# Monash-Connected-Autonomous-Vehicle/unsupervised-pseuso-LiDAR

Measured on AMD Instinct MI355X. Metric: images/sec (fwd+bwd) KITTI 192x640 triplets, full training step, higher is better.
Workload: dtype f32; 1 GPU; BASELINE.json configs[1]: per-GPU batch=12, 192x640 KITTI-shaped triplets, ResNet-18 depth encoder + 6-DoF PoseNet, fp32 (the ResNet trunk's 3x3 stride-1 convolutions and their data gradients: fp32 contractions on split operands -- three bf16 planes per operand, six bf16-MFMA plane products, fp32 accumulation; every other launch: fp32 MFMA), one step = 2x depth fwd + pose fwd + warp/L1/smooth loss; global_batch=12, parallelism=dp1

## Files before the change

### include/mcav_conv.h

```cpp
#ifndef MCAV_CONV_H
#define MCAV_CONV_H

#include <stddef.h>
#include <stdint.h>

#ifdef __cplusplus
extern "C" {
#endif

#define MCAV_G_DIRECT 0
#define MCAV_G_SMALLC 1
#define MCAV_G_ADJ_REFLECT 2
#define MCAV_G_ADJ_STRIDE2 3

#define MCAV_PAD_ZERO 0
#define MCAV_PAD_REFLECT 1

#define MCAV_ACT_NONE 0
#define MCAV_ACT_RELU 1
#define MCAV_ACT_ELU 2
#define MCAV_ACT_SIGMOID 3

#define MCAV_DACT_AFTER_ADDEND 0x100

// ... 35 lines not shown
    int B, Hs, Ws, C1, C2, up1;
    int kh, kw, Kp;
    int mode, stride, sign, offset, pad_mode;
    const float* dy;
    int Hd, Wd, Cdy, dy_choff;
    int Cout, Cin;
    float* dw_oihw;
    int accumulate;
    float* dbias;
    int tile;
    int upm, Cin_total, ci_offset;
    int mma;
} mcav_wgrad_desc;

size_t mcav_wgrad_workspace_bytes(const mcav_wgrad_desc* d);
int mcav_wgrad_uses_bf16(const mcav_wgrad_desc* d);
int mcav_wgrad(const mcav_wgrad_desc* d, void* workspace, size_t workspace_bytes, void* stream);

typedef struct mcav_wgrad_reduce_item {
    const float* slab;
    float* pre;
    float* dw;
    float* dbias;
    unsigned long long elems;
    int splits, groups, per_group, Ktot, slabN, Kp, taps, Cout, Cin, ci_t, accumulate, upm, cin_total, ci_off;
    int pre_bx, red_gx, red_gy, pre_first, red_first, reserved;
} mcav_wgrad_reduce_item;
int mcav_wgrad_deferred(const mcav_wgrad_desc* d, void* workspace, size_t workspace_bytes, mcav_wgrad_reduce_item* item, void* stream);
int mcav_wgrad_reduce_plan(mcav_wgrad_reduce_item* items, int n, int* presum_blocks, int* reduce_blocks, size_t* lds_bytes);
int mcav_wgrad_reduce_multi(const mcav_wgrad_reduce_item* items_dev, int n, int presum_blocks, int reduce_blocks, size_t lds_bytes, void* stream);

int mcav_pack_weights(const float* w_oihw, int Cout, int Cin, int kh, int kw, int transposed, float* packed, int Np, int Kp,
                      void* stream);

int mcav_pack_weights_multi(const void* items_dev, int nitems, int nblocks, void* stream);
int mcav_f32_to_bf16(const float* src, void* dst_bf16, size_t n, void* stream);
int mcav_f32_to_bf16_planes(const float* src, void* dst_bf16, size_t n, void* stream);
int mcav_pack_weights_blocks(int taps, int transposed, int Np, int Kp);
int mcav_pack_stem_weights(const float* w_oihw, int Cout, int Cin, float* packed, void* stream);
int mcav_pack_weights_upmerge(const float* w_oihw, int Cout, int Cin, int C1, float* packed, int Np, void* stream);
int mcav_pack_weights_upmerge_adj(const float* w_oihw, int Cout, int Cin, int C1, float* packed, int Np, int Kp, void* stream);
// ... 82 lines not shown
```

### unsupervised-pseuso-lidar_amd/csrc/conv_igemm.hip

```cpp
#include <stdlib.h>
#include <map>
#include <mutex>
#include <type_traits>
#include <utility>

#include "conv_shared.h"
#include "kernel_timer.h"

namespace mcav {

template <class T, int KIND>
__global__ __launch_bounds__(256) void igemm_kernel(IgemmParams p) {
    constexpr int BM = T::BM, BN = T::BN;
    constexpr int CK = T::KD;
    __shared__ __attribute__((aligned(16))) float As[2][BM][T::LD];
    __shared__ __attribute__((aligned(16))) float Bs[2][BN][T::LD];
    __shared__ int s_out[BM];
    __shared__ float s_stat[T::WAVES_M][2][BN];
    constexpr int MAXTAB = 9;
    __shared__ unsigned s_o1[KIND == K_GENERIC ? 1 : MAXTAB][KIND == K_GENERIC ? 1 : BM];
    __shared__ unsigned s_o2[KIND == K_GENERIC ? 1 : MAXTAB][KIND == K_GENERIC ? 1 : BM];
    __shared__ int s_rn[KIND == K_GENERIC ? 1 : BM], s_ry[KIND == K_GENERIC ? 1 : BM], s_rx[KIND == K_GENERIC ? 1 : BM];

    const int tid = threadIdx.x, lane = tid & 63, wave = tid >> 6;
// ... 1286 lines not shown
#pragma unroll
                for (int r = 0; r < T::ACC; ++r) {
                    const int dr = MF == 32 ? (r & 3) + 8 * (r >> 2) : r;
                    buf_store1(rslab, base + (unsigned)(dr * rowb), acc[i][j][r]);
                }
            }
        }
}

__device__ __forceinline__ void wgrad_presum_body(const float* slab, int splits, size_t elems, int per_group, float* dst, unsigned bx, unsigned by) {
    const size_t e4 = (size_t)bx * 256 + threadIdx.x;
    if (e4 * 4 >= elems) return;
    const int k0 = by * per_group, k1 = min(splits, k0 + per_group);
    const f32x4* src = reinterpret_cast<const f32x4*>(slab) + e4;
    const size_t stride4 = elems / 4;
    f32x4 s0 = {0.f, 0.f, 0.f, 0.f}, s1 = s0, s2 = s0, s3 = s0;
    int k = k0;
    for (; k + 3 < k1; k += 4) {
        s0 += src[(size_t)k * stride4];
        s1 += src[(size_t)(k + 1) * stride4];
        s2 += src[(size_t)(k + 2) * stride4];
        s3 += src[(size_t)(k + 3) * stride4];
    }
    for (; k < k1; ++k) s0 += src[(size_t)k * stride4];
    reinterpret_cast<f32x4*>(dst)[(size_t)by * stride4 + e4] = (s0 + s1) + (s2 + s3);
}

__global__ __launch_bounds__(256) void wgrad_presum_kernel(const float* slab, int splits, size_t elems, int per_group, float* dst) {
    wgrad_presum_body(slab, splits, elems, per_group, dst, blockIdx.x, blockIdx.y);
}

__device__ __forceinline__ void wgrad_reduce_body(float* lds, const float* slab, int splits, int Ktot, int slabN, int Kp, int taps, int Cout, int Cin,
                                                  int CI_T, float* dw, float* dbias, int accumulate, int upm, int Cin_total, int ci_off, int bx, int by) {
    const int co0 = bx * 32, ci0 = by * CI_T;
    const int tx = threadIdx.x & 31, ty = threadIdx.x >> 5;
    const int run = CI_T * taps, stride = run + 1;
    const size_t split_stride = (size_t)(Ktot + 1) * slabN;
    const bool col_ok = co0 + tx < slabN;
    if (upm) {
        for (int idx = ty; idx < run; idx += 8) {
            const int tap = idx / CI_T, r = idx - tap * CI_T, ci = ci0 + r;
            float sum = 0.f;
            if (ci < Cin && col_ok) {
                const int ky = tap / 3, kx = tap - ky * 3;
                for (int cls = 0; cls < 4; ++cls) {
                    const int py = cls >> 1, px = cls & 1;
                    const int ta = py == 0 ? (ky == 0 ? 0 : 1) : (ky == 2 ? 1 : 0), tb = px == 0 ? (kx == 0 ? 0 : 1) : (kx == 2 ? 1 : 0);
                    const float* src = slab + (size_t)((cls * 4 + ta * 2 + tb) * Kp + ci) * slabN + co0 + tx;
                    for (int k = 0; k < splits; ++k) sum += src[(size_t)k * split_stride];
                }
            }
            lds[tx * stride + r * taps + tap] = sum;
        }
    } else {
        for (int idx0 = ty; idx0 < run; idx0 += 32) {
            const float* src[4];
            float sum[4];
            int at[4];
#pragma unroll
            for (int u = 0; u < 4; ++u) {
                const int idx = idx0 + 8 * u, tap = idx / CI_T, r = idx - tap * CI_T;
                const bool ok = idx < run && ci0 + r < Cin && col_ok;
                src[u] = ok ? slab + (size_t)(tap * Kp + ci0 + r) * slabN + co0 + tx : nullptr;
                at[u] = idx < run ? tx * stride + r * taps + tap : -1;
                sum[u] = 0.f;
            }
            int k = 0;
            for (; k + 3 < splits; k += 4) {
                float v[4][4];
#pragma unroll
                for (int u = 0; u < 4; ++u)
#pragma unroll
                    for (int j = 0; j < 4; ++j) v[u][j] = src[u] ? src[u][(size_t)(k + j) * split_stride] : 0.f;
#pragma unroll
                for (int u = 0; u < 4; ++u)
#pragma unroll
                    for (int j = 0; j < 4; ++j) sum[u] += v[u][j];
            }
            for (; k < splits; ++k) {
#pragma unroll
                for (int u = 0; u < 4; ++u) sum[u] += src[u] ? src[u][(size_t)k * split_stride] : 0.f;
            }
#pragma unroll
            for (int u = 0; u < 4; ++u)
                if (at[u] >= 0) lds[at[u]] = sum[u];
        }
    }
    if (dbias && by == 0 && ty == 0 && co0 + tx < Cout) {
        const float* src = slab + (size_t)Ktot * slabN + co0 + tx;
        float sum = 0.f;
        for (int k = 0; k < splits; ++k) sum += src[(size_t)k * split_stride];
        dbias[co0 + tx] = accumulate ? dbias[co0 + tx] + sum : sum;
    }
    __syncthreads();
    const int valid_run = (Cin - ci0 < CI_T ? Cin - ci0 : CI_T) * taps;
    for (int e = threadIdx.x; e < 32 * run; e += 256) {
        const int col = e / run, q = e - col * run;
        if (co0 + col < Cout && q < valid_run) {
            const size_t o = ((size_t)(co0 + col) * Cin_total + ci_off + ci0) * taps + q;
            const float v = lds[col * stride + q];
            dw[o] = accumulate ? dw[o] + v : v;
        }
    }
}

__global__ __launch_bounds__(256) void wgrad_reduce_kernel(const float* slab, int splits, int Ktot, int slabN, int Kp, int taps, int Cout, int Cin,
                                                           int CI_T, float* dw, float* dbias, int accumulate, int upm, int Cin_total, int ci_off) {
    extern __shared__ float lds[];
    wgrad_reduce_body(lds, slab, splits, Ktot, slabN, Kp, taps, Cout, Cin, CI_T, dw, dbias, accumulate, upm, Cin_total, ci_off, blockIdx.x, blockIdx.y);
}

__device__ __forceinline__ int find_item(const mcav_wgrad_reduce_item* items, int n, int blk, bool presum) {
    int lo = 0;
    for (int i = 1; i < n; ++i)
        if ((presum ? items[i].pre_first : items[i].red_first) <= blk) lo = i;
    return lo;
}

__global__ __launch_bounds__(256) void wgrad_presum_multi_kernel(const mcav_wgrad_reduce_item* items, int n) {
    __shared__ int s_i;
    if (threadIdx.x == 0) {
        int best = -1;
        for (int i = 0; i < n; ++i)
            if (items[i].groups > 0 && items[i].pre_first <= (int)blockIdx.x) best = i;
        s_i = best;
    }
    __syncthreads();
    if (s_i < 0) return;
    const mcav_wgrad_reduce_item it = items[s_i];
    const int local = (int)blockIdx.x - it.pre_first;
    if (local >= it.pre_bx * it.groups) return;
    wgrad_presum_body(it.slab, it.splits, (size_t)it.elems, it.per_group, it.pre, (unsigned)(local % it.pre_bx), (unsigned)(local / it.pre_bx));
}

__global__ __launch_bounds__(256) void wgrad_reduce_multi_kernel(const mcav_wgrad_reduce_item* items, int n) {
    extern __shared__ float lds[];
    __shared__ int s_i;
    if (threadIdx.x == 0) s_i = find_item(items, n, (int)blockIdx.x, false);
    __syncthreads();
    const mcav_wgrad_reduce_item it = items[s_i];
    const int local = (int)blockIdx.x - it.red_first;
    if (local >= it.red_gx * it.red_gy) return;
    const float* src = it.groups > 0 ? it.pre : it.slab;
    wgrad_reduce_body(lds, src, it.groups > 0 ? it.groups : it.splits, it.Ktot, it.slabN, it.Kp, it.taps, it.Cout, it.Cin, it.ci_t, it.dw, it.dbias,
                      it.accumulate, it.upm, it.cin_total, it.ci_off, local % it.red_gx, local / it.red_gx);
}

__global__ void pack_weights_kernel(const float* w, int Cout, int Cin, int taps, int transposed, float* packed, int Np, int Kp, int Kstride) {
    const size_t total = (size_t)Np * Kstride;
    for (size_t e = (size_t)blockIdx.x * blockDim.x + threadIdx.x; e < total; e += (size_t)gridDim.x * blockDim.x) {
        const int n = (int)(e / Kstride), kf = (int)(e - (size_t)n * Kstride);
        const int tap = kf / Kp, k = kf - tap * Kp;
        float v = 0.f;
        if (tap < taps) {
            const int co = transposed ? k : n, ci = transposed ? n : k;
            if (co < Cout && ci < Cin) v = w[((size_t)co * Cin + ci) * taps + tap];
        }
        packed[e] = v;
    }
// ... 498 lines not shown
    const int wave_ch = T::BM / 4;
    const bool fast = (p.g.mode == MCAV_G_DIRECT || p.g.mode == MCAV_G_SMALLC) && (p.g.C1 & 3) == 0 && (p.g.C2 & 3) == 0 && (p.g.C2 == 0 || p.g.C1 % wave_ch == 0) &&
                      (p.CoutLoad & 3) == 0 && (p.Cdy & 3) == 0 && (p.dy_choff & 3) == 0 && p.Wd >= 16;
    if (fast) timed_launch(wgrad_kernel<T, K_FAST>, grid, dim3(256), 0, s, p);
    else timed_launch(wgrad_kernel<T, K_GENERIC>, grid, dim3(256), 0, s, p);
}

}

MCAV_EXPORT size_t mcav_wgrad_workspace_bytes(const mcav_wgrad_desc* d) {
    WgradPlan pl;
    if (!(d && d->mma != 0 && mcav_bf16_wgrad_plan(d, pl)) && !plan_wgrad(d, pl)) return 0;
    return pl.slab_bytes + pl.pre_bytes;
}

MCAV_EXPORT int mcav_wgrad_uses_bf16(const mcav_wgrad_desc* d) {
    WgradPlan pl;
    return d && d->mma != 0 && mcav_bf16_wgrad_plan(d, pl);
}

static int wgrad_gemm(const mcav_wgrad_desc* d, void* workspace, size_t workspace_bytes, hipStream_t s, WgradPlan& pl) {
    const bool bf16 = d && d->mma != 0 && mcav_bf16_wgrad_plan(d, pl);
    if ((!bf16 && !plan_wgrad(d, pl)) || !workspace) return MCAV_E_INVALID;
    if (workspace_bytes < pl.slab_bytes + pl.pre_bytes) return MCAV_E_WORKSPACE;
    const int cin_total = d->Cin_total > 0 ? d->Cin_total : d->Cin;
    if (d->ci_offset < 0 || d->ci_offset + d->Cin > cin_total) return MCAV_E_INVALID;
    pl.p.slab = reinterpret_cast<float*>(workspace);
    if (bf16) mcav_bf16_wgrad_launch(pl.p, s);
    else if (pl.use_stem) mcav_stem_wgrad_launch(d, pl.p.slab, pl.p.Ktot, pl.p.slabN, pl.p.splits, s);
    else if (pl.use_halo) mcav_halo_wgrad_launch(d, pl.p.slab, pl.p.slabN, pl.p.splits, s);
    else switch (pl.tile) {
        case 1: launch_wgrad<Tile128x64>(pl.p, pl.use_tab, s); break;
        case 2: launch_wgrad<Tile64x64>(pl.p, pl.use_tab, s); break;
        case 3: launch_wgrad<Tile256x32>(pl.p, pl.use_tab, s); break;
        case 4: launch_wgrad<Tile256x16>(pl.p, pl.use_tab, s); break;
        case 6: launch_wgrad<Tile64x16>(pl.p, pl.use_tab, s); break;
        case 7: launch_wgrad<Tile128x32>(pl.p, pl.use_tab, s); break;
        default: return MCAV_E_INVALID;
    }
    return MCAV_OK;
}

static void fill_reduce_item(const mcav_wgrad_desc* d, const WgradPlan& pl, void* workspace, mcav_wgrad_reduce_item& it) {
    it.slab = pl.p.slab;
    it.pre = pl.groups ? reinterpret_cast<float*>(reinterpret_cast<char*>(workspace) + pl.slab_bytes) : nullptr;
    it.dw = d->dw_oihw;
    it.dbias = d->dbias;
    it.elems = (unsigned long long)(pl.p.Ktot + 1) * pl.p.slabN;
    it.splits = pl.p.splits; it.groups = pl.groups; it.per_group = pl.per_group;
    it.Ktot = pl.p.Ktot; it.slabN = pl.p.slabN; it.Kp = pl.p.Kp;
    it.taps = pl.p.upm ? 9 : pl.p.taps;
    it.Cout = d->Cout; it.Cin = d->Cin; it.ci_t = pl.ci_t;
    it.accumulate = d->accumulate; it.upm = pl.p.upm;
    it.cin_total = d->Cin_total > 0 ? d->Cin_total : d->Cin;
    it.ci_off = d->ci_offset;
    it.pre_bx = pl.groups ? (int)((it.elems / 4 + 255) / 256) : 0;
    it.red_gx = (d->Cout + 31) / 32;
    it.red_gy = (d->Cin + pl.ci_t - 1) / pl.ci_t;
    it.pre_first = 0; it.red_first = 0;
}

MCAV_EXPORT int mcav_wgrad(const mcav_wgrad_desc* d, void* workspace, size_t workspace_bytes, void* stream) {
    WgradPlan pl;
    hipStream_t s = as_stream(stream);
    const int rc = wgrad_gemm(d, workspace, workspace_bytes, s, pl);
    if (rc != MCAV_OK) return rc;
    mcav_wgrad_reduce_item it;
    fill_reduce_item(d, pl, workspace, it);
    const size_t lds_bytes = sizeof(float) * 32 * (size_t)(it.ci_t * it.taps + 1);
    const float* rsrc = it.slab;
    int rsplits = it.splits;
    if (it.groups) {
        timed_launch(wgrad_presum_kernel, dim3((unsigned)it.pre_bx, it.groups), dim3(256), 0, s, (const float*)it.slab, it.splits, (size_t)it.elems,
                     it.per_group, it.pre);
        rsrc = it.pre;
        rsplits = it.groups;
    }
    timed_launch(wgrad_reduce_kernel, dim3(it.red_gx, it.red_gy), dim3(256), lds_bytes, s, rsrc, rsplits, it.Ktot, it.slabN, it.Kp, it.taps, it.Cout, it.Cin,
                 it.ci_t, it.dw, it.dbias, it.accumulate, it.upm, it.cin_total, it.ci_off);
    return launch_status();
}

MCAV_EXPORT int mcav_wgrad_deferred(const mcav_wgrad_desc* d, void* workspace, size_t workspace_bytes, mcav_wgrad_reduce_item* item, void* stream) {
    if (!item) return MCAV_E_INVALID;
    WgradPlan pl;
    const int rc = wgrad_gemm(d, workspace, workspace_bytes, as_stream(stream), pl);
    if (rc != MCAV_OK) return rc;
    fill_reduce_item(d, pl, workspace, *item);
    return launch_status();
}

MCAV_EXPORT int mcav_wgrad_reduce_plan(mcav_wgrad_reduce_item* items, int n, int* presum_blocks, int* reduce_blocks, size_t* lds_bytes) {
    if (!items || n <= 0 || !presum_blocks || !reduce_blocks || !lds_bytes) return MCAV_E_INVALID;
    int pb = 0, rb = 0;
    size_t lds = 0;
    for (int i = 0; i < n; ++i) {
        items[i].pre_first = pb;
        items[i].red_first = rb;
        pb += items[i].pre_bx * items[i].groups;
        rb += items[i].red_gx * items[i].red_gy;
        const size_t l = sizeof(float) * 32 * (size_t)(items[i].ci_t * items[i].taps + 1);
        if (l > lds) lds = l;
    }
    *presum_blocks = pb; *reduce_blocks = rb; *lds_bytes = lds;
    return MCAV_OK;
}

MCAV_EXPORT int mcav_wgrad_reduce_multi(const mcav_wgrad_reduce_item* items_dev, int n, int presum_blocks, int reduce_blocks, size_t lds_bytes, void* stream) {
    if (!items_dev || n <= 0 || reduce_blocks <= 0 || presum_blocks < 0) return MCAV_E_INVALID;
    hipStream_t s = as_stream(stream);
    if (presum_blocks > 0) timed_launch(wgrad_presum_multi_kernel, dim3(presum_blocks), dim3(256), 0, s, items_dev, n);
    timed_launch(wgrad_reduce_multi_kernel, dim3(reduce_blocks), dim3(256), lds_bytes, s, items_dev, n);
    return launch_status();
}

MCAV_EXPORT int mcav_pack_weights(const float* w_oihw, int Cout, int Cin, int kh, int kw, int transposed, float* packed, int Np, int Kp,
                                  void* stream) {
    if (!w_oihw || !packed || Cout <= 0 || Cin <= 0 || kh <= 0 || kw <= 0 || Np <= 0 || Kp <= 0) return MCAV_E_INVALID;
    if (!transposed && (Np < Cout || Kp < Cin)) return MCAV_E_INVALID;
    if (transposed && (Np < Cin || Kp < Cout)) return MCAV_E_INVALID;
    const int taps = kh * kw, Kstride = kstride_of(taps, Kp);
    const size_t total = (size_t)Np * Kstride;
    const int blocks = (int)((total + 255) / 256 < 2048 ? (total + 255) / 256 : 2048);
    pack_weights_kernel<<<blocks, 256, 0, as_stream(stream)>>>(w_oihw, Cout, Cin, taps, transposed, packed, Np, Kp, Kstride);
    return launch_status();
}
// ... 50 lines not shown
```

### unsupervised-pseuso-lidar_amd/csrc/warp_loss.hip

```cpp
#include <stdlib.h>
#include <mutex>
#include <type_traits>
#include <vector>

#include "mcav_common.h"
#include "kernel_timer.h"
#include "warp_math.h"

namespace mcav {

constexpr int TW = 32, TH = 8, HALO = 2, LW = TW + 2 * HALO, LH = TH + 2 * HALO;
constexpr int WL_SUB = 4, WLH = TH * WL_SUB, WL_LH = WLH + 2 * HALO;
constexpr int NACC = 38;
constexpr int SLAB = 40;

struct PrepConst {
    float Kf[9];
    SampleConst sc;
};

struct WLArgs {
    const float *tgt, *ref0, *ref1, *disp_t, *disp_r0, *poses;
    const void* K;
    const float* upstream;
// ... 594 lines not shown
    static const int xcd_align = MCAV_KNOB_INT("MCAV_WL_XCD", 1);
    if (xcd_align && G0 >= 8 && G1 >= 8) {
        int g0 = (G0 + 7) / 8 * 8, g1 = (G1 + 7) / 8 * 8;
        if ((g0 + g1) * B > slots) g1 = G1 / 8 * 8;
        if ((g0 + g1) * B > slots) g0 = G0 / 8 * 8;
        if (g0 >= 8 && g1 >= 8 && g0 <= ntiles && g1 <= ntiles && (g0 + g1) * B <= slots) { G0 = g0; G1 = g1; }
    }
}

inline dim3 pix_grid(int B, int H, int W) { return dim3((W + TW - 1) / TW, (H + TH - 1) / TH, B); }

}

using namespace mcav;

MCAV_EXPORT int mcav_abi_version(void) { return 1; }

MCAV_EXPORT size_t mcav_warp_loss_workspace_bytes(int B, int H, int W) {
    if (B <= 0 || H <= 0 || W <= 0) return 0;
    return ws_layout(B, H, W).total;
}

static std::mutex g_suspect_mu;
static std::vector<void*> g_suspect_ws;
static bool take_suspect(void* ws) {
    std::lock_guard<std::mutex> lk(g_suspect_mu);
    for (size_t i = 0; i < g_suspect_ws.size(); ++i)
        if (g_suspect_ws[i] == ws) { g_suspect_ws.erase(g_suspect_ws.begin() + i); return true; }
    return false;
}
static void mark_suspect(void* ws) {
// ... 247 lines not shown
```

### unsupervised-pseuso-lidar_amd/mcav/nn.py

```python
import ctypes
import os
import os as _os

import torch

from . import lib as L

c_p, c_i, c_f, c_sz, c_d = L.c_p, L.c_i, L.c_f, L.c_sz, ctypes.c_double

G_DIRECT, G_SMALLC, G_ADJ_REFLECT, G_ADJ_STRIDE2 = 0, 1, 2, 3
PAD_ZERO, PAD_REFLECT = 0, 1
ACT_NONE, ACT_RELU, ACT_ELU, ACT_SIGMOID = 0, 1, 2, 3
DACT_AFTER_ADDEND = 0x100


class IgemmDesc(ctypes.Structure):
    _fields_ = [("x1", c_p), ("x2", c_p), ("B", c_i), ("Hs", c_i), ("Ws", c_i), ("C1", c_i), ("C2", c_i), ("up1", c_i),
                ("w", c_p), ("kh", c_i), ("kw", c_i), ("Np", c_i), ("Kp", c_i),
                ("mode", c_i), ("stride", c_i), ("sign", c_i), ("offset", c_i), ("pad_mode", c_i),
                ("y", c_p), ("Hd", c_i), ("Wd", c_i), ("Cd", c_i), ("n_begin", c_i), ("n_count", c_i), ("y_choff", c_i),
                ("bias", c_p), ("act", c_i), ("dact_aux", c_p), ("dact", c_i), ("addend", c_p), ("pool", c_i), ("stats", c_p),
                ("tile", c_i), ("groups", c_i), ("w_upmerge", c_p), ("mma", c_i), ("w16", c_p),
                ("stats_x", c_p), ("stats_mean", c_p), ("stats_invstd", c_p), ("w_stem", c_p)]


class WgradDesc(ctypes.Structure):
    _fields_ = [("x1", c_p), ("x2", c_p), ("B", c_i), ("Hs", c_i), ("Ws", c_i), ("C1", c_i), ("C2", c_i), ("up1", c_i),
                ("kh", c_i), ("kw", c_i), ("Kp", c_i),
                ("mode", c_i), ("stride", c_i), ("sign", c_i), ("offset", c_i), ("pad_mode", c_i),
                ("dy", c_p), ("Hd", c_i), ("Wd", c_i), ("Cdy", c_i), ("dy_choff", c_i), ("Cout", c_i), ("Cin", c_i),
                ("dw_oihw", c_p), ("accumulate", c_i), ("dbias", c_p), ("tile", c_i), ("upm", c_i), ("Cin_total", c_i), ("ci_offset", c_i),
                ("mma", c_i)]


class WgradReduceItem(ctypes.Structure):
    _fields_ = [("slab", c_p), ("pre", c_p), ("dw", c_p), ("dbias", c_p), ("elems", ctypes.c_ulonglong)] + \
               [(n, c_i) for n in ("splits", "groups", "per_group", "Ktot", "slabN", "Kp", "taps", "Cout", "Cin", "ci_t", "accumulate", "upm", "cin_total",
                                   "ci_off", "pre_bx", "red_gx", "red_gy", "pre_first", "red_first", "reserved")]


L.register({
    "mcav_wgrad_deferred": (c_i, [ctypes.POINTER(WgradDesc), c_p, c_sz, ctypes.POINTER(WgradReduceItem), c_p]),
    "mcav_wgrad_reduce_plan": (c_i, [ctypes.POINTER(WgradReduceItem), c_i, ctypes.POINTER(c_i), ctypes.POINTER(c_i), ctypes.POINTER(c_sz)]),
    "mcav_wgrad_reduce_multi": (c_i, [c_p, c_i, c_i, c_i, c_sz, c_p]),
    "mcav_igemm_mtiles": (c_i, [ctypes.POINTER(IgemmDesc)]),
    "mcav_igemm": (c_i, [ctypes.POINTER(IgemmDesc), c_p]),
    "mcav_igemm_uses_bf16": (c_i, [ctypes.POINTER(IgemmDesc)]),
    "mcav_wgrad_uses_bf16": (c_i, [ctypes.POINTER(WgradDesc)]),
    "mcav_f32_to_bf16": (c_i, [c_p, c_p, c_sz, c_p]),
    "mcav_f32_to_bf16_planes": (c_i, [c_p, c_p, c_sz, c_p]),
    "mcav_pack_stem_weights": (c_i, [c_p, c_i, c_i, c_p, c_p]),
    "mcav_wgrad_workspace_bytes": (c_sz, [ctypes.POINTER(WgradDesc)]),
    "mcav_wgrad": (c_i, [ctypes.POINTER(WgradDesc), c_p, c_sz, c_p]),
    "mcav_pack_weights": (c_i, [c_p, c_i, c_i, c_i, c_i, c_i, c_p, c_i, c_i, c_p]),
    "mcav_pack_weights_multi": (c_i, [c_p, c_i, c_i, c_p]),
    "mcav_pack_weights_blocks": (c_i, [c_i, c_i, c_i, c_i]),
    "mcav_pack_weights_upmerge": (c_i, [c_p, c_i, c_i, c_i, c_p, c_i, c_p]),
    "mcav_pack_weights_upmerge_adj": (c_i, [c_p, c_i, c_i, c_i, c_p, c_i, c_i, c_p]),
    "mcav_upsample_adj_fold": (c_i, [c_p, c_i, c_i, c_i, c_i, c_p, c_i, c_p, c_p, c_p]),
    "mcav_nchw_to_nhwc": (c_i, [c_p, c_i, c_i, c_i, c_i, c_p, c_i, c_i, c_p]),
    "mcav_nchw3_to_nhwc": (c_i, [c_p, c_p, c_p, c_i, c_i, c_i, c_i, c_p, c_i, c_p]),
    "mcav_nhwc_to_nchw": (c_i, [c_p, c_i, c_i, c_i, c_i, c_i, c_i, c_p, c_p]),
    "mcav_bn_finalize": (c_i, [c_p, c_i, c_i, c_d, c_p, c_p, c_f, c_f] + [c_p] * 6 + [c_i, c_p, c_sz, c_p]),
    "mcav_bn_finalize_workspace_bytes": (c_sz, [c_i, c_i, c_i]),
    "mcav_bn_eval_coeffs": (c_i, [c_p, c_p, c_p, c_p, c_f, c_i, c_p, c_p, c_p]),
    "mcav_bn_apply": (c_i, [c_p, c_p, c_p, c_p, c_i, c_sz, c_i, c_p, c_sz, c_p]),
    "mcav_bn_bwd_workspace_bytes": (c_sz, [c_sz, c_i, c_i]),
# ... 588 lines not shown


def flush_wgrad_batch():
    if WGRAD_BATCH.items:
        if WGRAD_SIDE.forked:
            with torch.cuda.stream(WGRAD_SIDE.stream):
                WGRAD_BATCH.flush()
        else:
            WGRAD_BATCH.flush()


class _WgradBatch:

    def __init__(self):
        self.enabled = os.environ.get("MCAV_WGRAD_BATCH", "1") != "0"
        self.items = []
        self.targets = set()
        self.pool = {}
        self.tables = {}
        self.retired = []
        self.device = None

    def buffer(self, nbytes, device):
        k = (str(device), len(self.items))
        buf = self.pool.get(k)
        if buf is None or buf.numel() < nbytes:
            if buf is not None:
                self.retired.append(buf)
            buf = self.pool[k] = torch.empty(int(nbytes), dtype=torch.uint8, device=device)
        self.device = device
        return buf

    def flush(self):
        n = len(self.items)
        if n == 0:
            return
        arr = (WgradReduceItem * n)(*self.items)
        self.items = []
        self.targets = set()
        pb, rb, lds = c_i(0), c_i(0), c_sz(0)
        h = L.lib()
        L.check(h.mcav_wgrad_reduce_plan(arr, n, ctypes.byref(pb), ctypes.byref(rb), ctypes.byref(lds)), "mcav_wgrad_reduce_plan")
        key = (str(self.device), bytes(arr))
        hit = self.tables.get(key)
        if hit is None:
            if torch.cuda.is_current_stream_capturing():
                raise L.MCAVError("a batch of weight-gradient slab reductions was cut differently under hipGraph capture than in the warm-up step "
                                  "(its device table does not exist yet, and building it is a host -> device copy): warm-up and capture must "
                                  "announce the same gradient buckets (mcav/graph.py)")
            table = torch.frombuffer(bytearray(bytes(arr)), dtype=torch.uint8).to(self.device)
            hit = self.tables[key] = (table, pb.value, rb.value, lds.value)
        table, npb, nrb, nlds = hit
        with _Timed("wgrad", 0.0, "slab reduction of %d weight gradients (batched)" % n):
            L.check(h.mcav_wgrad_reduce_multi(P(table), n, npb, nrb, nlds, L.stream()), "mcav_wgrad_reduce_multi")


WGRAD_BATCH = _WgradBatch()


LAST_WGRAD_PLANES = 0


def launch_wgrad(d, tensors, flops=0.0, tag="", executed=None):
    h = L.lib()
    abytes = 4.0 * (sum(t.numel() for t in tensors if t is not None) + d.Cout * d.Cin * d.kh * d.kw)
    nbytes = h.mcav_wgrad_workspace_bytes(ctypes.byref(d))
    if nbytes == 0:
        raise L.MCAVError("mcav_wgrad: invalid descriptor")

    dev = tensors[0].device
    planes = _planes(d) if (d.mma and h.mcav_wgrad_uses_bf16(ctypes.byref(d))) else 0
    global LAST_WGRAD_PLANES
    LAST_WGRAD_PLANES = planes
    if planes:
        tag += _pipe_tag(d)
    defer = WGRAD_BATCH.enabled and dev.type == "cuda" and WGRAD_SIDE._note(torch.cuda.current_stream())
    if defer:
        target = (d.dw_oihw, d.ci_offset)
        if target in WGRAD_BATCH.targets:
            flush_wgrad_batch()
        WGRAD_BATCH.targets.add(target)
        ws = WGRAD_BATCH.buffer(nbytes, dev)
        item = WgradReduceItem()
        dd = WgradDesc.from_buffer_copy(d)

        def go_deferred():
            with _Timed("wgrad", flops, tag, executed, planes, abytes):
                L.check(h.mcav_wgrad_deferred(ctypes.byref(dd), P(ws), ws.numel(), ctypes.byref(item), L.stream()), "mcav_wgrad_deferred")
        WGRAD_SIDE.run(go_deferred, tensors)
        WGRAD_BATCH.items.append(item)
        return

    def go():
        ws = L.workspace(nbytes, dev, "wgrad")
        with _Timed("wgrad", flops, tag, executed, planes, abytes):
            L.check(h.mcav_wgrad(ctypes.byref(d), P(ws), ws.numel(), L.stream()), "mcav_wgrad")
# ... 244 lines not shown
```

Baseline: 1148 images/s.

## Fuse wgrad split-K presum and reduce into one-pass batched kernel

Adds a one-pass form of the batched weight-gradient slab reduction. Each wave sums groups of split-K partials and exchanges them through LDS, instead of running a separate presum kernel that writes and reads a pre-buffer. The reduce body also moves to float4 loads across columns, and items are sorted by cost before block assignment. This removes a launch and a global round-trip of partial sums. In exchange it uses more LDS per block, which may shrink the ci tile, and adds intra-wave exchange overhead.

```diff
diff --git a/include/mcav_conv.h b/include/mcav_conv.h
--- a/include/mcav_conv.h
+++ b/include/mcav_conv.h
@@ -73,6 +73,7 @@
 } mcav_wgrad_desc;
 
 size_t mcav_wgrad_workspace_bytes(const mcav_wgrad_desc* d);
+size_t mcav_wgrad_slab_bytes(const mcav_wgrad_desc* d);
 int mcav_wgrad_uses_bf16(const mcav_wgrad_desc* d);
 int mcav_wgrad(const mcav_wgrad_desc* d, void* workspace, size_t workspace_bytes, void* stream);
 
@@ -83,7 +84,7 @@
     float* dbias;
     unsigned long long elems;
     int splits, groups, per_group, Ktot, slabN, Kp, taps, Cout, Cin, ci_t, accumulate, upm, cin_total, ci_off;
-    int pre_bx, red_gx, red_gy, pre_first, red_first, reserved;
+    int pre_bx, red_gx, red_gy, pre_first, red_first, form;
 } mcav_wgrad_reduce_item;
 int mcav_wgrad_deferred(const mcav_wgrad_desc* d, void* workspace, size_t workspace_bytes, mcav_wgrad_reduce_item* item, void* stream);
 int mcav_wgrad_reduce_plan(mcav_wgrad_reduce_item* items, int n, int* presum_blocks, int* reduce_blocks, size_t* lds_bytes);
diff --git a/unsupervised-pseuso-lidar_amd/csrc/conv_igemm.hip b/unsupervised-pseuso-lidar_amd/csrc/conv_igemm.hip
--- a/unsupervised-pseuso-lidar_amd/csrc/conv_igemm.hip
+++ b/unsupervised-pseuso-lidar_amd/csrc/conv_igemm.hip
@@ -1,4 +1,5 @@
 #include <stdlib.h>
+#include <algorithm>
 #include <map>
 #include <mutex>
 #include <type_traits>
@@ -6,6 +7,7 @@
 
 #include "conv_shared.h"
 #include "kernel_timer.h"
+#include "wgrad_sum.h"
 
 namespace mcav {
 
@@ -1324,85 +1326,30 @@
     const int k0 = by * per_group, k1 = min(splits, k0 + per_group);
     const f32x4* src = reinterpret_cast<const f32x4*>(slab) + e4;
     const size_t stride4 = elems / 4;
-    f32x4 s0 = {0.f, 0.f, 0.f, 0.f}, s1 = s0, s2 = s0, s3 = s0;
-    int k = k0;
-    for (; k + 3 < k1; k += 4) {
-        s0 += src[(size_t)k * stride4];
-        s1 += src[(size_t)(k + 1) * stride4];
-        s2 += src[(size_t)(k + 2) * stride4];
-        s3 += src[(size_t)(k + 3) * stride4];
-    }
-    for (; k < k1; ++k) s0 += src[(size_t)k * stride4];
-    reinterpret_cast<f32x4*>(dst)[(size_t)by * stride4 + e4] = (s0 + s1) + (s2 + s3);
+    const f32x4 zero = {0.f, 0.f, 0.f, 0.f};
+    f32x4 part[1];
+    ws::group_partial<1>(part, zero, k0, k1, [&](int, int k) { return src[(size_t)k * stride4]; });
+    reinterpret_cast<f32x4*>(dst)[(size_t)by * stride4 + e4] = part[0];
 }
 
 __global__ __launch_bounds__(256) void wgrad_presum_kernel(const float* slab, int splits, size_t elems, int per_group, float* dst) {
     wgrad_presum_body(slab, splits, elems, per_group, dst, blockIdx.x, blockIdx.y);
 }
 
-__device__ __forceinline__ void wgrad_reduce_body(float* lds, const float* slab, int splits, int Ktot, int slabN, int Kp, int taps, int Cout, int Cin,
-                                                  int CI_T, float* dw, float* dbias, int accumulate, int upm, int Cin_total, int ci_off, int bx, int by) {
-    const int co0 = bx * 32, ci0 = by * CI_T;
-    const int tx = threadIdx.x & 31, ty = threadIdx.x >> 5;
-    const int run = CI_T * taps, stride = run + 1;
-    const size_t split_stride = (size_t)(Ktot + 1) * slabN;
-    const bool col_ok = co0 + tx < slabN;
-    if (upm) {
-        for (int idx = ty; idx < run; idx += 8) {
-            const int tap = idx / CI_T, r = idx - tap * CI_T, ci = ci0 + r;
-            float sum = 0.f;
-            if (ci < Cin && col_ok) {
-                const int ky = tap / 3, kx = tap - ky * 3;
-                for (int cls = 0; cls < 4; ++cls) {
-                    const int py = cls >> 1, px = cls & 1;
-                    const int ta = py == 0 ? (ky == 0 ? 0 : 1) : (ky == 2 ? 1 : 0), tb = px == 0 ? (kx == 0 ? 0 : 1) : (kx == 2 ? 1 : 0);
-                    const float* src = slab + (size_t)((cls * 4 + ta * 2 + tb) * Kp + ci) * slabN + co0 + tx;
-                    for (int k = 0; k < splits; ++k) sum += src[(size_t)k * split_stride];
-                }
-            }
-            lds[tx * stride + r * taps + tap] = sum;
-        }
-    } else {
-        for (int idx0 = ty; idx0 < run; idx0 += 32) {
-            const float* src[4];
-            float sum[4];
-            int at[4];
-#pragma unroll
-            for (int u = 0; u < 4; ++u) {
-                const int idx = idx0 + 8 * u, tap = idx / CI_T, r = idx - tap * CI_T;
-                const bool ok = idx < run && ci0 + r < Cin && col_ok;
-                src[u] = ok ? slab + (size_t)(tap * Kp + ci0 + r) * slabN + co0 + tx : nullptr;
-                at[u] = idx < run ? tx * stride + r * taps + tap : -1;
-                sum[u] = 0.f;
-            }
-            int k = 0;
-            for (; k + 3 < splits; k += 4) {
-                float v[4][4];
-#pragma unroll
-                for (int u = 0; u < 4; ++u)
-#pragma unroll
-                    for (int j = 0; j < 4; ++j) v[u][j] = src[u] ? src[u][(size_t)(k + j) * split_stride] : 0.f;
-#pragma unroll
-                for (int u = 0; u < 4; ++u)
-#pragma unroll
-                    for (int j = 0; j < 4; ++j) sum[u] += v[u][j];
-            }
-            for (; k < splits; ++k) {
-#pragma unroll
-                for (int u = 0; u < 4; ++u) sum[u] += src[u] ? src[u][(size_t)k * split_stride] : 0.f;
-            }
-#pragma unroll
-            for (int u = 0; u < 4; ++u)
-                if (at[u] >= 0) lds[at[u]] = sum[u];
-        }
-    }
-    if (dbias && by == 0 && ty == 0 && co0 + tx < Cout) {
-        const float* src = slab + (size_t)Ktot * slabN + co0 + tx;
-        float sum = 0.f;
-        for (int k = 0; k < splits; ++k) sum += src[(size_t)k * split_stride];
-        dbias[co0 + tx] = accumulate ? dbias[co0 + tx] + sum : sum;
-    }
-    __syncthreads();
+__device__ __forceinline__ int upm_row(int cls, int tap, int Kp, int ci) {
+    const int ky = tap / 3, kx = tap - ky * 3;
+    const int py = cls >> 1, px = cls & 1;
+    const int ta = py == 0 ? (ky == 0 ? 0 : 1) : (ky == 2 ? 1 : 0), tb = px == 0 ? (kx == 0 ? 0 : 1) : (kx == 2 ? 1 : 0);
+    return (cls * 4 + ta * 2 + tb) * Kp + ci;
+}
+
+__device__ __forceinline__ f32x4 ld4_or_zero(const float* p, size_t off) {
+    const f32x4 zero = {0.f, 0.f, 0.f, 0.f};
+    return p ? *reinterpret_cast<const f32x4*>(p + off) : zero;
+}
+
+__device__ __forceinline__ void wgrad_store_tile(const float* lds, int run, int stride, int co0, int ci0, int taps, int Cout, int Cin, int CI_T,
+                                                 float* dw, int accumulate, int Cin_total, int ci_off) {
     const int valid_run = (Cin - ci0 < CI_T ? Cin - ci0 : CI_T) * taps;
     for (int e = threadIdx.x; e < 32 * run; e += 256) {
         const int col = e / run, q = e - col * run;
@@ -1414,16 +1361,143 @@
     }
 }
 
+__device__ __forceinline__ void wgrad_reduce_body(float* lds, const float* slab, int splits, int Ktot, int slabN, int Kp, int taps, int Cout, int Cin,
+                                                  int CI_T, float* dw, float* dbias, int accumulate, int upm, int Cin_total, int ci_off, int bx, int by) {
+    const int co0 = bx * 32, ci0 = by * CI_T;
+    const int q4 = 4 * (threadIdx.x & 7), ty = threadIdx.x >> 3;
+    const int run = CI_T * taps, stride = run + 1;
+    const size_t split_stride = (size_t)(Ktot + 1) * slabN;
+    const bool col_ok = co0 + q4 < slabN;
+    const f32x4 zero = {0.f, 0.f, 0.f, 0.f};
+    if (upm) {
+        for (int idx = ty; idx < run; idx += 32) {
+            const int tap = idx / CI_T, r = idx - tap * CI_T, ci = ci0 + r;
+            f32x4 sum[1] = {zero};
+            if (ci < Cin && col_ok) {
+                for (int cls = 0; cls < 4; ++cls) {
+                    const float* src = slab + (size_t)upm_row(cls, tap, Kp, ci) * slabN + co0 + q4;
+                    ws::serial_add<1>(sum, splits, [&](int, int k) { return *reinterpret_cast<const f32x4*>(src + (size_t)k * split_stride); });
+                }
+            }
+#pragma unroll
+            for (int c = 0; c < 4; ++c) lds[(q4 + c) * stride + r * taps + tap] = sum[0][c];
+        }
+    } else {
+        for (int idx0 = ty; idx0 < run; idx0 += 128) {
+            const float* src[4];
+            f32x4 sum[4];
+            int at[4];
+#pragma unroll
+            for (int u = 0; u < 4; ++u) {
+                const int idx = idx0 + 32 * u, tap = idx / CI_T, r = idx - tap * CI_T;
+                const bool ok = idx < run && ci0 + r < Cin && col_ok;
+                src[u] = ok ? slab + (size_t)(tap * Kp + ci0 + r) * slabN + co0 + q4 : nullptr;
+                at[u] = idx < run ? q4 * stride + r * taps + tap : -1;
+                sum[u] = zero;
+            }
+            ws::serial_add<4>(sum, splits, [&](int u, int k) { return ld4_or_zero(src[u], (size_t)k * split_stride); });
+#pragma unroll
+            for (int u = 0; u < 4; ++u)
+                if (at[u] >= 0) {
+#pragma unroll
+                    for (int c = 0; c < 4; ++c) lds[at[u] + c * stride] = sum[u][c];
+                }
+        }
+    }
+    if (dbias && by == 0 && ty == 0 && col_ok) {
+        const float* src = slab + (size_t)Ktot * slabN + co0 + q4;
+        f32x4 sum[1] = {zero};
+        ws::serial_add<1>(sum, splits, [&](int, int k) { return *reinterpret_cast<const f32x4*>(src + (size_t)k * split_stride); });
+#pragma unroll
+        for (int c = 0; c < 4; ++c)
+            if (co0 + q4 + c < Cout) dbias[co0 + q4 + c] = accumulate ? dbias[co0 + q4 + c] + sum[0][c] : sum[0][c];
+    }
+    __syncthreads();
+    wgrad_store_tile(lds, run, stride, co0, ci0, taps, Cout, Cin, CI_T, dw, accumulate, Cin_total, ci_off);
+}
+
 __global__ __launch_bounds__(256) void wgrad_reduce_kernel(const float* slab, int splits, int Ktot, int slabN, int Kp, int taps, int Cout, int Cin,
                                                            int CI_T, float* dw, float* dbias, int accumulate, int upm, int Cin_total, int ci_off) {
     extern __shared__ float lds[];
     wgrad_reduce_body(lds, slab, splits, Ktot, slabN, Kp, taps, Cout, Cin, CI_T, dw, dbias, accumulate, upm, Cin_total, ci_off, blockIdx.x, blockIdx.y);
 }
 
-__device__ __forceinline__ int find_item(const mcav_wgrad_reduce_item* items, int n, int blk, bool presum) {
+constexpr int WG_XCH_FLOATS = 4 * 4 * 8 * 32;
+__device__ __forceinline__ void wgrad_onepass_body(float* xch_all, float* lds, const float* slab, int splits, int groups, int per_group, int Ktot,
+                                                   int slabN, int Kp, int taps, int Cout, int Cin, int CI_T, float* dw, float* dbias, int accumulate,
+                                                   int upm, int Cin_total, int ci_off, int bx, int by) {
+    const int co0 = bx * 32, ci0 = by * CI_T;
+    const int wave = threadIdx.x >> 6, lane = threadIdx.x & 63;
+    const int g = lane >> 3, q4 = 4 * (lane & 7);
+    const int run = CI_T * taps, stride = run + 1;
+    const size_t split_stride = (size_t)(Ktot + 1) * slabN;
+    const bool col_ok = co0 + q4 < slabN;
+    const int k0 = g * per_group, k1 = min(splits, k0 + per_group);
+    const f32x4 zero = {0.f, 0.f, 0.f, 0.f};
+    float* xch = xch_all + wave * (4 * 8 * 32);
+    auto exchange = [&](const float* const (&src)[4]) {
+        f32x4 part[4];
+        ws::group_partial<4>(part, zero, k0, k1, [&](int u, int k) { return ld4_or_zero(src[u], (size_t)k * split_stride); });
+        __builtin_amdgcn_fence(__ATOMIC_ACQ_REL, "wavefront");
+        __builtin_amdgcn_wave_barrier();
+#pragma unroll
+        for (int u = 0; u < 4; ++u) *reinterpret_cast<f32x4*>(xch + (u * 8 + g) * 32 + q4) = part[u];
+        __builtin_amdgcn_fence(__ATOMIC_ACQ_REL, "wavefront");
+        __builtin_amdgcn_wave_barrier();
+    };
+    if (upm) {
+        for (int idx = wave; idx < run; idx += 4) {
+            const int tap = idx / CI_T, r = idx - tap * CI_T, ci = ci0 + r;
+            const float* src[4];
+#pragma unroll
+            for (int cls = 0; cls < 4; ++cls)
+                src[cls] = ci < Cin && col_ok ? slab + (size_t)upm_row(cls, tap, Kp, ci) * slabN + co0 + q4 : nullptr;
+            exchange(src);
+            if (lane < 32) {
+                float sum = 0.f;
+                for (int cls = 0; cls < 4; ++cls)
+                    for (int gg = 0; gg < groups; ++gg) sum += xch[(cls * 8 + gg) * 32 + lane];
+                lds[lane * stride + r * taps + tap] = sum;
+            }
+        }
+    } else {
+        for (int idx0 = 4 * wave; idx0 < run; idx0 += 16) {
+            const float* src[4];
+#pragma unroll
+            for (int u = 0; u < 4; ++u) {
+                const int idx = idx0 + u, tap = idx / CI_T, r = idx - tap * CI_T;
+                src[u] = idx < run && ci0 + r < Cin && col_ok ? slab + (size_t)(tap * Kp + ci0 + r) * slabN + co0 + q4 : nullptr;
+            }
+            exchange(src);
+#pragma unroll
+            for (int j = 0; j < 2; ++j) {
+                const int u = (lane >> 5) + 2 * j, col = lane & 31, idx = idx0 + u;
+                float sum = 0.f;
+                for (int gg = 0; gg < groups; ++gg) sum += xch[(u * 8 + gg) * 32 + col];
+                if (idx < run) {
+                    const int tap = idx / CI_T, r = idx - tap * CI_T;
+                    lds[col * stride + r * taps + tap] = sum;
+                }
+            }
+        }
+    }
+    if (dbias && by == 0 && wave == 0) {
+        const float* src[4] = {col_ok ? slab + (size_t)Ktot * slabN + co0 + q4 : nullptr, nullptr, nullptr, nullptr};
+        exchange(src);
+        if (lane < 32 && co0 + lane < Cout) {
+            float sum = 0.f;
+            for (int gg = 0; gg < groups; ++gg) sum += xch[gg * 32 + lane];
+            dbias[co0 + lane] = accumulate ? dbias[co0 + lane] + sum : sum;
+        }
+    }
+    __syncthreads();
+    wgrad_store_tile(lds, run, stride, co0, ci0, taps, Cout, Cin, CI_T, dw, accumulate, Cin_total, ci_off);
+}
+
+__device__ __forceinline__ int find_item(const mcav_wgrad_reduce_item* items, int n, int blk) {
     int lo = 0;
     for (int i = 1; i < n; ++i)
-        if ((presum ? items[i].pre_first : items[i].red_first) <= blk) lo = i;
+        if (items[i].red_first <= blk) lo = i;
     return lo;
 }
 
@@ -1432,7 +1506,7 @@
     if (threadIdx.x == 0) {
         int best = -1;
         for (int i = 0; i < n; ++i)
-            if (items[i].groups > 0 && items[i].pre_first <= (int)blockIdx.x) best = i;
+            if (items[i].groups > 0 && items[i].form == 0 && items[i].pre_first <= (int)blockIdx.x) best = i;
         s_i = best;
     }
     __syncthreads();
@@ -1446,13 +1520,19 @@
 __global__ __launch_bounds__(256) void wgrad_reduce_multi_kernel(const mcav_wgrad_reduce_item* items, int n) {
     extern __shared__ float lds[];
     __shared__ int s_i;
-    if (threadIdx.x == 0) s_i = find_item(items, n, (int)blockIdx.x, false);
+    if (threadIdx.x == 0) s_i = find_item(items, n, (int)blockIdx.x);
     __syncthreads();
     const mcav_wgrad_reduce_item it = items[s_i];
     const int local = (int)blockIdx.x - it.red_first;
     if (local >= it.red_gx * it.red_gy) return;
+    float* tile = lds + WG_XCH_FLOATS;
+    if (it.groups > 0 && it.form == 1) {
+        wgrad_onepass_body(lds, tile, it.slab, it.splits, it.groups, it.per_group, it.Ktot, it.slabN, it.Kp, it.taps, it.Cout, it.Cin, it.ci_t, it.dw,
+                           it.dbias, it.accumulate, it.upm, it.cin_total, it.ci_off, local % it.red_gx, local / it.red_gx);
+        return;
+    }
     const float* src = it.groups > 0 ? it.pre : it.slab;
-    wgrad_reduce_body(lds, src, it.groups > 0 ? it.groups : it.splits, it.Ktot, it.slabN, it.Kp, it.taps, it.Cout, it.Cin, it.ci_t, it.dw, it.dbias,
+    wgrad_reduce_body(tile, src, it.groups > 0 ? it.groups : it.splits, it.Ktot, it.slabN, it.Kp, it.taps, it.Cout, it.Cin, it.ci_t, it.dw, it.dbias,
                       it.accumulate, it.upm, it.cin_total, it.ci_off, local % it.red_gx, local / it.red_gx);
 }
 
@@ -1981,15 +2061,21 @@
     return pl.slab_bytes + pl.pre_bytes;
 }
 
+MCAV_EXPORT size_t mcav_wgrad_slab_bytes(const mcav_wgrad_desc* d) {
+    WgradPlan pl;
+    if (!(d && d->mma != 0 && mcav_bf16_wgrad_plan(d, pl)) && !plan_wgrad(d, pl)) return 0;
+    return pl.slab_bytes;
+}
+
 MCAV_EXPORT int mcav_wgrad_uses_bf16(const mcav_wgrad_desc* d) {
     WgradPlan pl;
     return d && d->mma != 0 && mcav_bf16_wgrad_plan(d, pl);
 }
 
-static int wgrad_gemm(const mcav_wgrad_desc* d, void* workspace, size_t workspace_bytes, hipStream_t s, WgradPlan& pl) {
+static int wgrad_gemm(const mcav_wgrad_desc* d, void* workspace, size_t workspace_bytes, hipStream_t s, WgradPlan& pl, bool need_pre) {
     const bool bf16 = d && d->mma != 0 && mcav_bf16_wgrad_plan(d, pl);
     if ((!bf16 && !plan_wgrad(d, pl)) || !workspace) return MCAV_E_INVALID;
-    if (workspace_bytes < pl.slab_bytes + pl.pre_bytes) return MCAV_E_WORKSPACE;
+    if (workspace_bytes < pl.slab_bytes + (need_pre ? pl.pre_bytes : 0)) return MCAV_E_WORKSPACE;
     const int cin_total = d->Cin_total > 0 ? d->Cin_total : d->Cin;
     if (d->ci_offset < 0 || d->ci_offset + d->Cin > cin_total) return MCAV_E_INVALID;
     pl.p.slab = reinterpret_cast<float*>(workspace);
@@ -2008,9 +2094,9 @@
     return MCAV_OK;
 }
 
-static void fill_reduce_item(const mcav_wgrad_desc* d, const WgradPlan& pl, void* workspace, mcav_wgrad_reduce_item& it) {
+static void fill_reduce_item(const mcav_wgrad_desc* d, const WgradPlan& pl, void* workspace, bool has_pre, mcav_wgrad_reduce_item& it) {
     it.slab = pl.p.slab;
-    it.pre = pl.groups ? reinterpret_cast<float*>(reinterpret_cast<char*>(workspace) + pl.slab_bytes) : nullptr;
+    it.pre = pl.groups && has_pre ? reinterpret_cast<float*>(reinterpret_cast<char*>(workspace) + pl.slab_bytes) : nullptr;
     it.dw = d->dw_oihw;
     it.dbias = d->dbias;
     it.elems = (unsigned long long)(pl.p.Ktot + 1) * pl.p.slabN;
@@ -2024,16 +2110,16 @@
     it.pre_bx = pl.groups ? (int)((it.elems / 4 + 255) / 256) : 0;
     it.red_gx = (d->Cout + 31) / 32;
     it.red_gy = (d->Cin + pl.ci_t - 1) / pl.ci_t;
-    it.pre_first = 0; it.red_first = 0;
+    it.pre_first = 0; it.red_first = 0; it.form = 0;
 }
 
 MCAV_EXPORT int mcav_wgrad(const mcav_wgrad_desc* d, void* workspace, size_t workspace_bytes, void* stream) {
     WgradPlan pl;
     hipStream_t s = as_stream(stream);
-    const int rc = wgrad_gemm(d, workspace, workspace_bytes, s, pl);
+    const int rc = wgrad_gemm(d, workspace, workspace_bytes, s, pl, true);
     if (rc != MCAV_OK) return rc;
     mcav_wgrad_reduce_item it;
-    fill_reduce_item(d, pl, workspace, it);
+    fill_reduce_item(d, pl, workspace, true, it);
     const size_t lds_bytes = sizeof(float) * 32 * (size_t)(it.ci_t * it.taps + 1);
     const float* rsrc = it.slab;
     int rsplits = it.splits;
@@ -2051,32 +2137,58 @@
 MCAV_EXPORT int mcav_wgrad_deferred(const mcav_wgrad_desc* d, void* workspace, size_t workspace_bytes, mcav_wgrad_reduce_item* item, void* stream) {
     if (!item) return MCAV_E_INVALID;
     WgradPlan pl;
-    const int rc = wgrad_gemm(d, workspace, workspace_bytes, as_stream(stream), pl);
+    const int rc = wgrad_gemm(d, workspace, workspace_bytes, as_stream(stream), pl, false);
     if (rc != MCAV_OK) return rc;
-    fill_reduce_item(d, pl, workspace, *item);
+    fill_reduce_item(d, pl, workspace, workspace_bytes >= pl.slab_bytes + pl.pre_bytes, *item);
     return launch_status();
+}
+
+static long reduce_block_cost(const mcav_wgrad_reduce_item& it) {
+    const long rows = (long)it.ci_t * (it.upm ? 16 : it.taps);
+    const int walked = it.groups > 0 && it.form == 0 ? it.groups : it.splits;
+    return rows * walked;
 }
 
 MCAV_EXPORT int mcav_wgrad_reduce_plan(mcav_wgrad_reduce_item* items, int n, int* presum_blocks, int* reduce_blocks, size_t* lds_bytes) {
     if (!items || n <= 0 || !presum_blocks || !reduce_blocks || !lds_bytes) return MCAV_E_INVALID;
+    for (int i = 0; i < n; ++i) {
+        mcav_wgrad_reduce_item& it = items[i];
+        if (it.slabN & 3) return MCAV_E_INVALID;
+        if (it.form != 0 && it.form != 1) return MCAV_E_INVALID;
+        if (it.groups == 0) it.form = 0;
+        if (it.groups > 8) return MCAV_E_INVALID;
+        if (it.groups > 0 && it.form == 0 && !it.pre) return MCAV_E_WORKSPACE;
+        if (it.form == 1) { it.pre = nullptr; it.pre_bx = 0; }
+    }
+    const size_t xch = sizeof(float) * WG_XCH_FLOATS;
+    size_t lds = 0;
+    for (int i = 0; i < n; ++i) {
+        mcav_wgrad_reduce_item& it = items[i];
+        while (it.ci_t > 1 && xch + sizeof(float) * 32 * (size_t)(it.ci_t * it.taps + 1) > 65536) it.ci_t >>= 1;
+        it.red_gy = (it.Cin + it.ci_t - 1) / it.ci_t;
+        const size_t l = xch + sizeof(float) * 32 * (size_t)(it.ci_t * it.taps + 1);
+        if (l > 65536) return MCAV_E_INVALID;
+        if (l > lds) lds = l;
+    }
+    std::stable_sort(items, items + n, [](const mcav_wgrad_reduce_item& a, const mcav_wgrad_reduce_item& b) {
+        return reduce_block_cost(a) > reduce_block_cost(b);
+    });
     int pb = 0, rb = 0;
-    size_t lds = 0;
     for (int i = 0; i < n; ++i) {
         items[i].pre_first = pb;
         items[i].red_first = rb;
-        pb += items[i].pre_bx * items[i].groups;
+        pb += items[i].pre_bx * (items[i].form == 0 ? items[i].groups : 0);
         rb += items[i].red_gx * items[i].red_gy;
-        const size_t l = sizeof(float) * 32 * (size_t)(items[i].ci_t * items[i].taps + 1);
-        if (l > lds) lds = l;
     }
     *presum_blocks = pb; *reduce_blocks = rb; *lds_bytes = lds;
     return MCAV_OK;
 }
 
 MCAV_EXPORT int mcav_wgrad_reduce_multi(const mcav_wgrad_reduce_item* items_dev, int n, int presum_blocks, int reduce_blocks, size_t lds_bytes, void* stream) {
-    if (!items_dev || n <= 0 || reduce_blocks <= 0 || presum_blocks < 0) return MCAV_E_INVALID;
+    if (!items_dev || n <= 0 || reduce_blocks <= 0 || presum_blocks < 0 || lds_bytes > 65536) return MCAV_E_INVALID;
     hipStream_t s = as_stream(stream);
     if (presum_blocks > 0) timed_launch(wgrad_presum_multi_kernel, dim3(presum_blocks), dim3(256), 0, s, items_dev, n);
+    if (lds_bytes <= sizeof(float) * WG_XCH_FLOATS) return MCAV_E_INVALID;
     timed_launch(wgrad_reduce_multi_kernel, dim3(reduce_blocks), dim3(256), lds_bytes, s, items_dev, n);
     return launch_status();
 }
diff --git a/unsupervised-pseuso-lidar_amd/csrc/warp_loss.hip b/unsupervised-pseuso-lidar_amd/csrc/warp_loss.hip
--- a/unsupervised-pseuso-lidar_amd/csrc/warp_loss.hip
+++ b/unsupervised-pseuso-lidar_amd/csrc/warp_loss.hip
@@ -632,7 +632,7 @@
 
 using namespace mcav;
 
-MCAV_EXPORT int mcav_abi_version(void) { return 1; }
+MCAV_EXPORT int mcav_abi_version(void) { return 2; }
 
 MCAV_EXPORT size_t mcav_warp_loss_workspace_bytes(int B, int H, int W) {
     if (B <= 0 || H <= 0 || W <= 0) return 0;
diff --git a/unsupervised-pseuso-lidar_amd/csrc/wgrad_sum.h b/unsupervised-pseuso-lidar_amd/csrc/wgrad_sum.h
--- /dev/null
+++ b/unsupervised-pseuso-lidar_amd/csrc/wgrad_sum.h
@@ -0,0 +1,93 @@
+#pragma once
+
+#if defined(__HIPCC__)
+#define MCAV_WS_HD __host__ __device__ __forceinline__
+#else
+#define MCAV_WS_HD inline
+#endif
+
+namespace mcav {
+namespace ws {
+
+constexpr int MAX_DIRECT = 8;
+constexpr int MAX_GROUPS = 8;
+
+MCAV_WS_HD int groups_of(int splits) {
+    if (splits <= MAX_DIRECT) return 0;
+    const int per_group = (splits + MAX_GROUPS - 1) / MAX_GROUPS;
+    return (splits + per_group - 1) / per_group;
+}
+MCAV_WS_HD int per_group_of(int splits) { return splits <= MAX_DIRECT ? 0 : (splits + MAX_GROUPS - 1) / MAX_GROUPS; }
+
+template <int U, class V, class Load>
+MCAV_WS_HD void serial_add(V (&sum)[U], int n, Load ld) {
+    int k = 0;
+    for (; k + 3 < n; k += 4) {
+        V v[U][4];
+#pragma unroll
+        for (int u = 0; u < U; ++u)
+#pragma unroll
+            for (int j = 0; j < 4; ++j) v[u][j] = ld(u, k + j);
+#pragma unroll
+        for (int u = 0; u < U; ++u)
+#pragma unroll
+            for (int j = 0; j < 4; ++j) sum[u] += v[u][j];
+    }
+    for (; k < n; ++k) {
+        V v[U];
+#pragma unroll
+        for (int u = 0; u < U; ++u) v[u] = ld(u, k);
+#pragma unroll
+        for (int u = 0; u < U; ++u) sum[u] += v[u];
+    }
+}
+
+template <int U, class V, class Load>
+MCAV_WS_HD void group_partial(V (&out)[U], V zero, int k0, int k1, Load ld) {
+    V s0[U], s1[U], s2[U], s3[U];
+#pragma unroll
+    for (int u = 0; u < U; ++u) s0[u] = s1[u] = s2[u] = s3[u] = zero;
+    int k = k0;
+    for (; k + 3 < k1; k += 4) {
+        V v[U][4];
+#pragma unroll
+        for (int u = 0; u < U; ++u)
+#pragma unroll
+            for (int j = 0; j < 4; ++j) v[u][j] = ld(u, k + j);
+#pragma unroll
+        for (int u = 0; u < U; ++u) {
+            s0[u] += v[u][0];
+            s1[u] += v[u][1];
+            s2[u] += v[u][2];
+            s3[u] += v[u][3];
+        }
+    }
+    for (; k < k1; ++k) {
+        V v[U];
+#pragma unroll
+        for (int u = 0; u < U; ++u) v[u] = ld(u, k);
+#pragma unroll
+        for (int u = 0; u < U; ++u) s0[u] += v[u];
+    }
+#pragma unroll
+    for (int u = 0; u < U; ++u) out[u] = (s0[u] + s1[u]) + (s2[u] + s3[u]);
+}
+
+template <int U, class V, class Load>
+MCAV_WS_HD void onepass_add(V (&sum)[U], V zero, int splits, Load ld) {
+    const int groups = groups_of(splits), per_group = per_group_of(splits);
+    if (groups == 0) {
+        serial_add<U>(sum, splits, ld);
+        return;
+    }
+    for (int g = 0; g < groups; ++g) {
+        const int k0 = g * per_group, k1 = splits < k0 + per_group ? splits : k0 + per_group;
+        V part[U];
+        group_partial<U>(part, zero, k0, k1, ld);
+#pragma unroll
+        for (int u = 0; u < U; ++u) sum[u] += part[u];
+    }
+}
+
+}
+}
diff --git a/unsupervised-pseuso-lidar_amd/mcav/nn.py b/unsupervised-pseuso-lidar_amd/mcav/nn.py
--- a/unsupervised-pseuso-lidar_amd/mcav/nn.py
+++ b/unsupervised-pseuso-lidar_amd/mcav/nn.py
@@ -36,7 +36,7 @@
 class WgradReduceItem(ctypes.Structure):
     _fields_ = [("slab", c_p), ("pre", c_p), ("dw", c_p), ("dbias", c_p), ("elems", ctypes.c_ulonglong)] + \
                [(n, c_i) for n in ("splits", "groups", "per_group", "Ktot", "slabN", "Kp", "taps", "Cout", "Cin", "ci_t", "accumulate", "upm", "cin_total",
-                                   "ci_off", "pre_bx", "red_gx", "red_gy", "pre_first", "red_first", "reserved")]
+                                   "ci_off", "pre_bx", "red_gx", "red_gy", "pre_first", "red_first", "form")]
 
 
 L.register({
@@ -51,6 +51,7 @@
     "mcav_f32_to_bf16_planes": (c_i, [c_p, c_p, c_sz, c_p]),
     "mcav_pack_stem_weights": (c_i, [c_p, c_i, c_i, c_p, c_p]),
     "mcav_wgrad_workspace_bytes": (c_sz, [ctypes.POINTER(WgradDesc)]),
+    "mcav_wgrad_slab_bytes": (c_sz, [ctypes.POINTER(WgradDesc)]),
     "mcav_wgrad": (c_i, [ctypes.POINTER(WgradDesc), c_p, c_sz, c_p]),
     "mcav_pack_weights": (c_i, [c_p, c_i, c_i, c_i, c_i, c_i, c_p, c_i, c_i, c_p]),
     "mcav_pack_weights_multi": (c_i, [c_p, c_i, c_i, c_p]),
@@ -669,6 +670,8 @@
 
     def __init__(self):
         self.enabled = os.environ.get("MCAV_WGRAD_BATCH", "1") != "0"
+        self.onepass = os.environ.get("MCAV_WGRAD_ONEPASS", "1") != "0"
+        self.last_plan = None
         self.items = []
         self.targets = set()
         self.pool = {}
@@ -691,6 +694,8 @@
         if n == 0:
             return
         arr = (WgradReduceItem * n)(*self.items)
+        for i in range(n):
+            arr[i].form = int(self.onepass)
         self.items = []
         self.targets = set()
         pb, rb, lds = c_i(0), c_i(0), c_sz(0)
@@ -706,6 +711,7 @@
             table = torch.frombuffer(bytearray(bytes(arr)), dtype=torch.uint8).to(self.device)
             hit = self.tables[key] = (table, pb.value, rb.value, lds.value)
         table, npb, nrb, nlds = hit
+        self.last_plan = (npb, nrb, nlds)
         with _Timed("wgrad", 0.0, "slab reduction of %d weight gradients (batched)" % n):
             L.check(h.mcav_wgrad_reduce_multi(P(table), n, npb, nrb, nlds, L.stream()), "mcav_wgrad_reduce_multi")
 
@@ -735,6 +741,8 @@
         if target in WGRAD_BATCH.targets:
             flush_wgrad_batch()
         WGRAD_BATCH.targets.add(target)
+        if WGRAD_BATCH.onepass:
+            nbytes = h.mcav_wgrad_slab_bytes(ctypes.byref(d))
         ws = WGRAD_BATCH.buffer(nbytes, dev)
         item = WgradReduceItem()
         dd = WgradDesc.from_buffer_copy(d)
```

Result: no change. 1153 images/s (median of 6 runs) (+0.4%).
